# Snoworday/instance-segmentation-attention

Hardware: AMD Instinct MI355X
Metric: images/sec @256x256 bs=16 per GPU (higher is better)
Workload: dtype bf16; 1 GPU; train.py step fwd+bwd+update 256x256 bs=16/GPU (bf16); global_batch=16, parallelism=dp1, launch=hipGraph replay

## Files before the change

### instance-segmentation-attention_amd/csrc/common.hpp

```cpp
#pragma once
#include <hip/hip_runtime.h>
#include <stdint.h>
#include "../../include/isa_kernels.h"

typedef __bf16 bf16_t;
typedef __bf16 bf16x8 __attribute__((ext_vector_type(8)));
typedef __bf16 bf16x4 __attribute__((ext_vector_type(4)));
typedef float f32x4 __attribute__((ext_vector_type(4)));
typedef float f32x16 __attribute__((ext_vector_type(16)));

#define ISA_WAVE 64
#define ISA_STAT_R 8

static inline hipStream_t as_stream(void* s) { return reinterpret_cast<hipStream_t>(s); }

static inline int launch_status() {
    return hipGetLastError() == hipSuccess ? ISA_OK : ISA_ELAUNCH;
}

static inline bool tensor_ok(const isa_tensor* t, int align_elems) {
    if (!t || !t->data || t->n <= 0 || t->h <= 0 || t->w <= 0 || t->c <= 0 || t->ld < t->c) return false;
    if (t->dtype != ISA_F32 && t->dtype != ISA_BF16) return false;
    if (align_elems > 1) {
        size_t esz = t->dtype == ISA_F32 ? 4 : 2;
        if ((reinterpret_cast<uintptr_t>(t->data) % (align_elems * esz)) != 0) return false;
        if (t->ld % align_elems) return false;
    }
    return true;
}

template <typename T> struct st;
template <> struct st<float> {
    static constexpr int dtype = ISA_F32;
    static __device__ __forceinline__ float ld(const float* p) { return *p; }
    static __device__ __forceinline__ void stv(float* p, float v) { *p = v; }
};
template <> struct st<bf16_t> {
    static constexpr int dtype = ISA_BF16;
    static __device__ __forceinline__ float ld(const bf16_t* p) { return (float)*p; }
    static __device__ __forceinline__ void stv(bf16_t* p, float v) { *p = (bf16_t)v; }
};

template <typename T> __device__ __forceinline__ void load8(const T* p, float (&v)[8]);
template <> __device__ __forceinline__ void load8<float>(const float* p, float (&v)[8]) {
    f32x4 a = *reinterpret_cast<const f32x4*>(p), b = *reinterpret_cast<const f32x4*>(p + 4);
#pragma unroll
    for (int i = 0; i < 4; ++i) { v[i] = a[i]; v[4 + i] = b[i]; }
}
template <> __device__ __forceinline__ void load8<bf16_t>(const bf16_t* p, float (&v)[8]) {
    bf16x8 a = *reinterpret_cast<const bf16x8*>(p);
#pragma unroll
    for (int i = 0; i < 8; ++i) v[i] = (float)a[i];
}
template <typename T> __device__ __forceinline__ void store8(T* p, const float (&v)[8]);
template <> __device__ __forceinline__ void store8<float>(float* p, const float (&v)[8]) {
    f32x4 a, b;
#pragma unroll
    for (int i = 0; i < 4; ++i) { a[i] = v[i]; b[i] = v[4 + i]; }
    *reinterpret_cast<f32x4*>(p) = a;
    *reinterpret_cast<f32x4*>(p + 4) = b;
}
template <> __device__ __forceinline__ void store8<bf16_t>(bf16_t* p, const float (&v)[8]) {
    bf16x8 a;
#pragma unroll
    for (int i = 0; i < 8; ++i) a[i] = (bf16_t)v[i];
    *reinterpret_cast<bf16x8*>(p) = a;
}

template <typename T> __device__ __forceinline__ void load8g(const T* p, float (&v)[8], int nv) {
    if (nv >= 8) { load8<T>(p, v); return; }
#pragma unroll
    for (int i = 0; i < 8; ++i) v[i] = i < nv ? st<T>::ld(p + i) : 0.f;
}
template <typename T> __device__ __forceinline__ void store8g(T* p, const float (&v)[8], int nv) {
    if (nv >= 8) { store8<T>(p, v); return; }
#pragma unroll
    for (int i = 0; i < 8; ++i) if (i < nv) st<T>::stv(p + i, v[i]);
}

template <int CLS> __device__ __forceinline__ float row_fold(float v) {
    static_assert(CLS == 4 || CLS == 8, "lane classes per row");
    if constexpr (CLS == 4) v += __int_as_float(__builtin_amdgcn_update_dpp(0, __float_as_int(v), 0x124, 0xF, 0xF, false));
    v += __int_as_float(__builtin_amdgcn_update_dpp(0, __float_as_int(v), 0x128, 0xF, 0xF, false));
    return v;
}

__device__ __forceinline__ float act_apply(float z, int act) {
    switch (act) {
        case ISA_ACT_RELU:  return fmaxf(z, 0.f);
        case ISA_ACT_RELU6: return fminf(fmaxf(z, 0.f), 6.f);
        case ISA_ACT_LEAKY: return z > 0.f ? z : 0.01f * z;
        case ISA_ACT_TANH:  return tanhf(z);
        default:            return z;
    }
}
__device__ __forceinline__ float act_grad(float z, int act) {
    switch (act) {
        case ISA_ACT_RELU:  return z > 0.f ? 1.f : 0.f;
        case ISA_ACT_RELU6: return (z > 0.f && z < 6.f) ? 1.f : 0.f;
        case ISA_ACT_LEAKY: return z > 0.f ? 1.f : 0.01f;
        case ISA_ACT_TANH:  { float t = tanhf(z); return 1.f - t * t; }
        default:            return 1.f;
    }
}

constexpr int ACT_RT = -1;
template <int ACT> __device__ __forceinline__ float act_t(float z, int rt) {
    if constexpr (ACT == ISA_ACT_RELU6) return __builtin_amdgcn_fmed3f(z, 0.f, 6.f);
    else if constexpr (ACT == ISA_ACT_NONE) return z;
    else if constexpr (ACT == ISA_ACT_LEAKY) return z > 0.f ? z : 0.01f * z;
    else return act_apply(z, rt);
}
template <int ACT> __device__ __forceinline__ float act_grad_t(float z, int rt) {
    if constexpr (ACT == ISA_ACT_RELU6) return (z > 0.f && z < 6.f) ? 1.f : 0.f;
    else if constexpr (ACT == ISA_ACT_NONE) return 1.f;
    else if constexpr (ACT == ISA_ACT_LEAKY) return z > 0.f ? 1.f : 0.01f;
    else return act_grad(z, rt);
}

struct ProDev {
    const float* scale; const float* shift; const float* bscale; int act;
};
static inline ProDev make_pro(const isa_pro* p) {
    ProDev d{nullptr, nullptr, nullptr, ISA_ACT_NONE};
    if (p) { d.scale = p->scale; d.shift = p->shift; d.bscale = p->bscale; d.act = p->act; }
    return d;
}
static inline bool pro_trivial(const ProDev& p) {
    return !p.scale && !p.shift && !p.bscale && p.act == ISA_ACT_NONE;
}

struct FinDev {
    const float *stats, *gamma, *beta; float *rm, *rv, *scale, *shift, *mean, *invstd;
    float count, momentum, eps; int repeat;
};
static inline FinDev make_fin(const isa_pro* p) {
    FinDev f{}; f.repeat = 1;
    if (p && p->fin) {
        const isa_bn_fin* q = p->fin;
        f = FinDev{q->stats, q->gamma, q->beta, q->running_mean, q->running_var, q->scale, q->shift, q->mean, q->invstd,
                   q->count, q->momentum, q->eps, q->repeat < 1 ? 1 : q->repeat};
    }
    return f;
}
static inline bool fin_valid(const isa_pro* p) {
    return !p || !p->fin || (p->fin->stats && p->fin->scale && p->fin->shift && p->fin->scale == p->scale && p->fin->shift == p->shift);
}
int fin_standalone(const isa_pro* p, int c, int groups, hipStream_t s);

__device__ __forceinline__ void bn_fin_channel(const FinDev& f, int i, int c, int groups, bool all_groups, int gsel,
                                               float* tab, int tab_ld) {
    const float g = f.gamma ? f.gamma[i] : 1.f, b = f.beta ? f.beta[i] : 0.f;
    const bool run = all_groups || !f.stats;
    float rmi = (run && f.rm) ? f.rm[i] : 0.f, rvi = (run && f.rv) ? f.rv[i] : 0.f;
    const int g0 = all_groups ? 0 : gsel, g1 = all_groups ? groups : gsel + 1;
    for (int gi = g0; gi < g1; ++gi) {
        float mean, var;
        if (f.stats) {
            const float* st = f.stats + (long)gi * ISA_STAT_R * 2 * c;
            float s1 = 0.f, s2 = 0.f;
// ... 115 lines not shown
```

### instance-segmentation-attention_amd/csrc/dwconv.hip

```cpp
#include "common.hpp"
#include <type_traits>

namespace {

__device__ __forceinline__ void lds_barrier() {
    __builtin_amdgcn_fence(__ATOMIC_RELEASE, "workgroup", "local");
    __builtin_amdgcn_s_barrier();
    __builtin_amdgcn_fence(__ATOMIC_ACQUIRE, "workgroup", "local");
}

constexpr int TH = 8, TW = 32, CB = 32, PS = 36;
constexpr int HALO = (TH + 2) * (TW + 2);

struct Dw2Params {
    const void* x; const void* w; const float* bias; void* y; const void* dy;
    int n, h, w_, c, ldx, ldy, ldd, wld;
    ProDev pro;
    float* stats; int accumulate;
    int tiles_x, tiles_y; long ntiles;
    float* ws; int csrc;
    int G;
    FinDev fin;
};

template <typename T> struct raw8;
template <> struct raw8<bf16_t> {
    bf16x8 v;
    __device__ __forceinline__ void load(const bf16_t* p) { v = *reinterpret_cast<const bf16x8*>(p); }
    __device__ __forceinline__ float get(int j) const { return (float)v[j]; }
    __device__ __forceinline__ void store(bf16_t* p) const { *reinterpret_cast<bf16x8*>(p) = v; }
    __device__ __forceinline__ void zero() { v = bf16x8{}; }
};
template <> struct raw8<float> {
    f32x4 a, b;
    __device__ __forceinline__ void load(const float* p) { a = *reinterpret_cast<const f32x4*>(p); b = *reinterpret_cast<const f32x4*>(p + 4); }
    __device__ __forceinline__ float get(int j) const { return j < 4 ? a[j] : b[j - 4]; }
    __device__ __forceinline__ void store(float* p) const { *reinterpret_cast<f32x4*>(p) = a; *reinterpret_cast<f32x4*>(p + 4) = b; }
    __device__ __forceinline__ void zero() { a = f32x4{}; b = f32x4{}; }
};

struct ProRegs { float sc[8], sh[8], bs[8]; };

template <bool HAS_PRO>
__device__ __forceinline__ void load_pro(const Dw2Params& p, ProRegs& r, int c0, int b) {
#pragma unroll
    for (int j = 0; j < 8; ++j) {
        const int c = min(c0 + j, p.c - 1);
        r.sc[j] = (HAS_PRO && p.pro.scale) ? p.pro.scale[c] : 1.f;
        r.sh[j] = (HAS_PRO && p.pro.shift) ? p.pro.shift[c] : 0.f;
        r.bs[j] = (HAS_PRO && p.pro.bscale) ? p.pro.bscale[(long)b * p.c + c] : 1.f;
    }
}

template <typename T, bool HAS_PRO, int ACT>
__device__ __forceinline__ void stage_tile(const Dw2Params& p, const ProRegs& r, float* tile, int b, int ty, int tx, int c_base) {
    const T* xin = reinterpret_cast<const T*>(p.x);
    const int cg = threadIdx.x & 3;
    const int c0 = c_base + cg * 8;
    const bool cok = c0 < p.c;
    constexpr int NIT = (HALO * 4 + 255) / 256;
    float v[NIT][8];
    bool ok[NIT];
#pragma unroll
    for (int it = 0; it < NIT; ++it) {
        const int pix = (threadIdx.x + it * 256) >> 2;
        const int rr = pix / (TW + 2), cc = pix - rr * (TW + 2);
        const int gy = ty * TH + rr - 1, gx = tx * TW + cc - 1;
        ok[it] = pix < HALO && cok && gy >= 0 && gy < p.h && gx >= 0 && gx < p.w_;
        if (ok[it]) load8<T>(xin + (((long)b * p.h + gy) * p.w_ + gx) * p.ldx + c0, v[it]);
    }
#pragma unroll
    for (int it = 0; it < NIT; ++it) {
        const int pix = (threadIdx.x + it * 256) >> 2;
        if (pix >= HALO) continue;
        f32x4 a, bb;
#pragma unroll
        for (int j = 0; j < 8; ++j) {
            float z = 0.f;
            if (ok[it]) {
                z = v[it][j];
                if constexpr (HAS_PRO) {
                    z = act_t<ACT>(fmaf(z, r.sc[j], r.sh[j]), p.pro.act);
                    if (p.pro.bscale) z *= r.bs[j];
                }
            }
            if (j < 4) a[j] = z; else bb[j - 4] = z;
        }
        *reinterpret_cast<f32x4*>(tile + pix * PS + cg * 8) = a;
        *reinterpret_cast<f32x4*>(tile + pix * PS + cg * 8 + 4) = bb;
    }
}

typedef float f32x2 __attribute__((ext_vector_type(2)));
__device__ __forceinline__ void fma8(const float (&x)[8], const float (&w)[8], float (&acc)[8]) {
#ifdef ISA_DW_SCALAR_FMA
#pragma unroll
    for (int j = 0; j < 8; ++j) acc[j] = __builtin_fmaf(x[j], w[j], acc[j]);
#else
#pragma unroll
    for (int j = 0; j < 8; j += 2) {
        const f32x2 r = __builtin_elementwise_fma(f32x2{x[j], x[j + 1]}, f32x2{w[j], w[j + 1]}, f32x2{acc[j], acc[j + 1]});
        acc[j] = r[0]; acc[j + 1] = r[1];
    }
#endif
}

__device__ __forceinline__ void ld8(const float* p, float (&v)[8]) {
    const f32x4 a = *reinterpret_cast<const f32x4*>(p), b = *reinterpret_cast<const f32x4*>(p + 4);
#pragma unroll
    for (int j = 0; j < 4; ++j) { v[j] = a[j]; v[4 + j] = b[j]; }
}

struct TileRange { long t0, end, step; };
__device__ __forceinline__ TileRange tile_range(long ntiles, int bx, int nbx) {
    if ((nbx & 7) == 0 && ntiles >= 64) {
        const int xcd = bx & 7, j = bx >> 3;
        const long chunk = (ntiles + 7) / 8;
        const long end = min(ntiles, (xcd + 1) * chunk);
        return TileRange{xcd * chunk + j, end, (long)(nbx >> 3)};
    }
    return TileRange{(long)bx, ntiles, (long)nbx};
}
// ... 885 lines not shown
```

### instance-segmentation-attention_amd/csrc/elementwise.hip

```cpp
#include "common.hpp"

namespace {

template <typename T>
__global__ void pack_kernel(const isa_pack_entry* tab, const int32_t* kmap, const float* src, T* dst) {
    const isa_pack_entry e = tab[blockIdx.y];
    const float* s = src + e.src_off;
    T* d = dst + e.dst_off;
    const int32_t* km = e.kmap_off >= 0 ? kmap + e.kmap_off : nullptr;
    long total;
    const int rows = e.rows;
    switch (e.kind) {
        case 0: case 1: total = (long)rows * e.taps * e.kp; break;
        case 2: total = (long)rows * e.kp; break;
        case 3: total = (long)rows * 4 * e.kp; break;
        default: total = (long)9 * rows; break;
    }
    for (long i = (long)blockIdx.x * blockDim.x + threadIdx.x; i < total; i += (long)gridDim.x * blockDim.x) {
        float v = 0.f;
        if (e.kind == 0) {
            const int kd = (int)(i % e.kp); long q = i / e.kp;
            const int t = (int)(q % e.taps); const int n = (int)(q / e.taps);
            const int k = km ? km[kd] : (kd < e.k ? kd : -1);
            if (k >= 0) v = s[((long)n * e.k + k) * e.taps + t];
        } else if (e.kind == 1) {
            const int nd = (int)(i % e.kp); long q = i / e.kp;
            const int t = (int)(q % e.taps); const int kd = (int)(q / e.taps);
            const int k = km ? km[kd] : kd;
            if (k >= 0 && nd < e.n) v = s[((long)nd * e.k + k) * e.taps + (e.taps - 1 - t)];
        } else if (e.kind == 2) {
            const int kd = (int)(i % e.kp); const int row = (int)(i / e.kp);
            const int co_n = e.n;
            const int qd = row / co_n, co = row - qd * co_n;
            const int k = km ? km[kd] : (kd < e.k ? kd : -1);
            if (k >= 0) v = s[((long)k * co_n + co) * 4 + qd];
        } else if (e.kind == 3) {
            const int cod = (int)(i % e.kp); long q = i / e.kp;
            const int qd = (int)(q % 4); const int kd = (int)(q / 4);
            const int k = km ? km[kd] : kd;
            if (k >= 0 && cod < e.n) v = s[((long)k * e.n + cod) * 4 + qd];
        } else {
            const int cd = (int)(i % rows); const int t = (int)(i / rows);
            const int c = km ? km[cd] : (cd < e.n ? cd : -1);
            if (c >= 0) v = s[(long)c * 9 + (e.kind == 5 ? 8 - t : t)];
        }
        d[i] = (T)v;
    }
}

__global__ void bn_finalize_kernel(FinDev f, int c, int groups) {
    for (int i = blockIdx.x * blockDim.x + threadIdx.x; i < c; i += gridDim.x * blockDim.x)
        bn_fin_channel(f, i, c, groups, true, 0, nullptr, 0);
}

constexpr int BN_UPD_CHUNK = 64;
struct BnUpdChunk { isa_bn_upd d[BN_UPD_CHUNK]; };
__global__ __launch_bounds__(256) void bn_running_update_kernel(BnUpdChunk ch, float momentum) {
    const isa_bn_upd u = ch.d[blockIdx.x];
    const int c = u.c;
    for (int i = threadIdx.x; i < c; i += 256) {
        float s1 = 0.f, s2 = 0.f;
#pragma unroll
        for (int r = 0; r < ISA_STAT_R; ++r) { s1 += u.stats[r * 2 * c + i]; s2 += u.stats[r * 2 * c + c + i]; }
        const float mean = s1 / u.count;
        const float var = fmaxf(s2 / u.count - mean * mean, 0.f);
        u.running_mean[i] = (1.f - momentum) * u.running_mean[i] + momentum * mean;
        u.running_var[i] = (1.f - momentum) * u.running_var[i] + momentum * var * (u.count / fmaxf(u.count - 1.f, 1.f));
    }
}

struct View { void* data; int n, h, w, c, ld; };
static inline View mkview(const isa_tensor* t) { return View{t->data, t->n, t->h, t->w, t->c, t->ld}; }

struct BnBwdParams {
    View dt, y, dy;
    const float *scale, *shift, *mean, *invstd, *bscale, *gamma, *red;
    float* out_red; float* dgamma; float* dbeta;
    float inv_count; int act, train;
    long pixels; int cg;
    int groups;
};

struct Walk { int cg, sh; long pixels; };
static inline Walk mkwalk(int c, long pixels) {
    Walk w; w.cg = (c + 7) / 8; w.sh = 0;
    while ((1 << w.sh) < w.cg) ++w.sh;
    if (w.sh > 8) w.sh = 8;
    w.pixels = pixels; return w;
}
static inline int walk_grid(const Walk& w, int iters = 1) { return grid_cap(cdiv(w.pixels, (long)(256 >> w.sh) * iters)); }

template <typename T, bool APPLY, int ACT>
__global__ __launch_bounds__(256) void bn_bwd_kernel(BnBwdParams p, Walk wk) {
    extern __shared__ float red[];
    const int C = p.y.c;
    if (p.groups > 1 && blockIdx.z) {
        const long g = blockIdx.z, gp = g * wk.pixels;
        p.dt.data = reinterpret_cast<T*>(p.dt.data) + gp * p.dt.ld;
        p.y.data = reinterpret_cast<T*>(p.y.data) + gp * p.y.ld;
        if (APPLY) p.dy.data = reinterpret_cast<T*>(p.dy.data) + gp * p.dy.ld;
        p.scale = goff(p.scale, g * C); p.shift = goff(p.shift, g * C); p.mean = goff(p.mean, g * C);
        p.invstd = goff(p.invstd, g * C);
        p.bscale = goff(p.bscale, g * (wk.pixels / ((long)p.y.h * p.y.w)) * C);
        p.red = goff(p.red, g * ISA_STAT_R * 2 * C); p.out_red = goff(p.out_red, g * ISA_STAT_R * 2 * C);
    }
    if (!APPLY) {
        for (int i = threadIdx.x; i < 2 * C; i += 256) red[i] = 0.f;
        __syncthreads();
    } else if (p.red) {
        const int cw = 8 << wk.sh;
        for (int cb = blockIdx.y * cw; cb < C; cb += gridDim.y * cw) {
            for (int i = threadIdx.x; i < 2 * cw; i += 256) {
                const int which = i / cw, c = cb + (i - which * cw);
                if (c >= C) continue;
                float s = 0.f;
#pragma unroll
                for (int r = 0; r < ISA_STAT_R; ++r) s += p.red[r * 2 * C + which * C + c];
                red[which * C + c] = s;
                if (blockIdx.x == 0) {
                    if (which == 1 && p.dgamma) atomicAdd(p.dgamma + c, s);
                    if (which == 0 && p.dbeta) atomicAdd(p.dbeta + c, s);
                }
            }
        }
        __syncthreads();
    }
    const int ppb = 256 >> wk.sh;
    const int psub = threadIdx.x >> wk.sh;
    const unsigned hw = (unsigned)p.y.h * (unsigned)p.y.w;
    for (int cgi = (blockIdx.y << wk.sh) + (threadIdx.x & ((1 << wk.sh) - 1)); cgi < wk.cg; cgi += (gridDim.y << wk.sh)) {
        const int c0 = cgi * 8;
        const int nv = min(8, C - c0);
        float sc[8], sh[8], mu[8], is[8], k0[8], k1[8], s0[8], s1[8];
#pragma unroll
        for (int j = 0; j < 8; ++j) {
            const int c = min(c0 + j, C - 1);
            sc[j] = p.scale ? p.scale[c] : 1.f;
            sh[j] = p.shift ? p.shift[c] : 0.f;
            mu[j] = p.mean ? p.mean[c] : 0.f;
            is[j] = p.invstd ? p.invstd[c] : 1.f;
            k0[j] = (APPLY && p.train) ? red[c] * p.inv_count : 0.f;
            k1[j] = (APPLY && p.train) ? red[C + c] * p.inv_count : 0.f;
            s0[j] = 0.f; s1[j] = 0.f;
        }
        const long step = (long)gridDim.x * ppb;
        for (long pix = (long)blockIdx.x * ppb + psub; pix < wk.pixels; pix += step) {
            float dt[8], yv[8], out[8];
            load8g<T>(reinterpret_cast<const T*>(p.dt.data) + pix * p.dt.ld + c0, dt, nv);
            load8g<T>(reinterpret_cast<const T*>(p.y.data) + pix * p.y.ld + c0, yv, nv);
            const float* bs = p.bscale ? p.bscale + (long)((unsigned)pix / hw) * C : nullptr;
#pragma unroll
            for (int j = 0; j < 8; ++j) {
                const float z = fmaf(yv[j], sc[j], sh[j]);
                float dz = dt[j] * act_grad_t<ACT>(z, p.act);
                if (bs) dz *= bs[min(c0 + j, C - 1)];
                const float yh = (yv[j] - mu[j]) * is[j];
                if (!APPLY) { s0[j] += dz; s1[j] += dz * yh; }
                else out[j] = sc[j] * (dz - k0[j] - yh * k1[j]);
            }
            if (APPLY) store8g<T>(reinterpret_cast<T*>(p.dy.data) + pix * p.dy.ld + c0, out, nv);
        }
        if (!APPLY) {
            const int lane = threadIdx.x & 63;
            if (wk.sh < 6) {
#pragma unroll
                for (int j = 0; j < 8; ++j) {
                    for (int off = 1 << wk.sh; off < 64; off <<= 1) {
                        s0[j] += __shfl_xor(s0[j], off, 64); s1[j] += __shfl_xor(s1[j], off, 64);
                    }
                }
            }
            if (wk.sh >= 6 || (lane >> wk.sh) == 0) {
#pragma unroll
                for (int j = 0; j < 8; ++j)
                    if (j < nv) { atomicAdd(&red[c0 + j], s0[j]); atomicAdd(&red[C + c0 + j], s1[j]); }
            }
        }
    }
    if (!APPLY) {
        __syncthreads();
        float* rep = p.out_red + (blockIdx.x & (ISA_STAT_R - 1)) * 2 * C;
        for (int i = threadIdx.x; i < 2 * C; i += 256)
            if (red[i] != 0.f) atomicAdd(rep + i, red[i]);
    }
}

struct MatParams { View x, res, res2, out; ProDev pro; const float* oscale; long pixels; int cg; int has_res, has_res2; int groups, bcast; FinDev fin; };
template <typename T, int ACT>
__global__ __launch_bounds__(256) void materialize_kernel(MatParams p, Walk wk) {
    const int C = p.x.c;
    __shared__ float fin_tab[2 * ISA_FIN_MAX_C];
    const bool fin = bn_fin_inline<256>(p.fin, C, p.bcast ? 1 : p.groups, p.bcast ? 0 : (int)blockIdx.z, fin_tab, ISA_FIN_MAX_C,
                                        threadIdx.x);
    if (p.groups > 1 && blockIdx.z) {
        const long g = blockIdx.z, gp = g * wk.pixels;
        const long gimg = g * (wk.pixels / ((long)p.x.h * p.x.w)) * C;
        p.out.data = reinterpret_cast<T*>(p.out.data) + gp * p.out.ld;
        if (p.has_res2) p.res2.data = reinterpret_cast<T*>(p.res2.data) + gp * p.res2.ld;
        p.oscale = goff(p.oscale, gimg);
        if (!p.bcast) {
            p.x.data = reinterpret_cast<T*>(p.x.data) + gp * p.x.ld;
            if (p.has_res) p.res.data = reinterpret_cast<T*>(p.res.data) + gp * p.res.ld;
            p.pro.scale = goff(p.pro.scale, g * C); p.pro.shift = goff(p.pro.shift, g * C);
            p.pro.bscale = goff(p.pro.bscale, gimg);
        }
    }
    const int ppb = 256 >> wk.sh;
    const int psub = threadIdx.x >> wk.sh;
    const unsigned hw = (unsigned)p.x.h * (unsigned)p.x.w;
    for (int cgi = threadIdx.x & ((1 << wk.sh) - 1); cgi < wk.cg; cgi += (1 << wk.sh)) {
        const int c0 = cgi * 8;
        const int nv = min(8, C - c0);
        float sc[8], sh[8];
#pragma unroll
        for (int j = 0; j < 8; ++j) {
            const int c = min(c0 + j, C - 1);
            sc[j] = fin ? fin_tab[c] : (p.pro.scale ? p.pro.scale[c] : 1.f);
            sh[j] = fin ? fin_tab[ISA_FIN_MAX_C + c] : (p.pro.shift ? p.pro.shift[c] : 0.f);
        }
        const bool per_image = p.pro.bscale || p.oscale;
        const long step = (long)gridDim.x * ppb;
        for (long pix = (long)blockIdx.x * ppb + psub; pix < wk.pixels; pix += step) {
            float v[8];
            load8g<T>(reinterpret_cast<const T*>(p.x.data) + pix * p.x.ld + c0, v, nv);
            const long bofs = per_image ? (long)((unsigned)pix / hw) * C : 0;
#pragma unroll
            for (int j = 0; j < 8; ++j) v[j] = act_t<ACT>(fmaf(v[j], sc[j], sh[j]), p.pro.act);
            if (p.pro.bscale) {
#pragma unroll
                for (int j = 0; j < 8; ++j) v[j] *= p.pro.bscale[bofs + min(c0 + j, C - 1)];
            }
            if (p.has_res) {
                float rr[8];
                load8g<T>(reinterpret_cast<const T*>(p.res.data) + pix * p.res.ld + c0, rr, nv);
#pragma unroll
                for (int j = 0; j < 8; ++j) v[j] += rr[j];
            }
            if (p.has_res2) {
                float rr[8];
                load8g<T>(reinterpret_cast<const T*>(p.res2.data) + pix * p.res2.ld + c0, rr, nv);
#pragma unroll
                for (int j = 0; j < 8; ++j) v[j] += rr[j];
            }
            if (p.oscale) {
#pragma unroll
                for (int j = 0; j < 8; ++j) v[j] *= p.oscale[bofs + min(c0 + j, C - 1)];
            }
            store8g<T>(reinterpret_cast<T*>(p.out.data) + pix * p.out.ld + c0, v, nv);
        }
    }
}

struct AxpyParams { View src, dst; float alpha; int accumulate; long pixels; };
template <typename T>
__global__ __launch_bounds__(256) void axpy_kernel(AxpyParams p) {
    const int C = p.src.c;
    const long items = p.pixels * C;
    for (long i = (long)blockIdx.x * 256 + threadIdx.x; i < items; i += (long)gridDim.x * 256) {
        const int c = (int)(i % C); const long pix = i / C;
        float v = p.alpha == 0.f ? 0.f : p.alpha * st<T>::ld(reinterpret_cast<const T*>(p.src.data) + pix * p.src.ld + c);
        T* d = reinterpret_cast<T*>(p.dst.data) + pix * p.dst.ld + c;
        if (p.accumulate) v += st<T>::ld(d);
        st<T>::stv(d, v);
    }
}
template <typename T>
__global__ __launch_bounds__(256) void axpy8_kernel(AxpyParams p) {
    const int cg = p.src.c / 8;
    const long items = p.pixels * cg;
    for (long i = (long)blockIdx.x * 256 + threadIdx.x; i < items; i += (long)gridDim.x * 256) {
        const int c0 = (int)(i % cg) * 8; const long pix = i / cg;
        float v[8] = {0, 0, 0, 0, 0, 0, 0, 0};
        if (p.alpha != 0.f) load8<T>(reinterpret_cast<const T*>(p.src.data) + pix * p.src.ld + c0, v);
        T* d = reinterpret_cast<T*>(p.dst.data) + pix * p.dst.ld + c0;
        if (p.accumulate) {
            float o[8]; load8<T>(d, o);
#pragma unroll
            for (int j = 0; j < 8; ++j) v[j] = fmaf(p.alpha, v[j], o[j]);
        } else {
#pragma unroll
            for (int j = 0; j < 8; ++j) v[j] *= p.alpha;
        }
        store8<T>(d, v);
    }
}

struct PoolParams { View x, y; int accumulate; };
template <typename T, bool BWD>
__global__ __launch_bounds__(256) void avgpool2_kernel(PoolParams p) {
    const View big = BWD ? p.y : p.x, small = BWD ? p.x : p.y;
    const int cg = small.c / 8;
    const long items = (long)small.n * small.h * small.w * cg;
    for (long i = (long)blockIdx.x * 256 + threadIdx.x; i < items; i += (long)gridDim.x * 256) {
        const int c0 = (int)(i % cg) * 8; long q = i / cg;
        const int xs = (int)(q % small.w); q /= small.w;
        const int ys = (int)(q % small.h); const int b = (int)(q / small.h);
        T* sp = reinterpret_cast<T*>(small.data) + (((long)b * small.h + ys) * small.w + xs) * small.ld + c0;
        T* bp = reinterpret_cast<T*>(big.data) + (((long)b * big.h + 2 * ys) * big.w + 2 * xs) * big.ld + c0;
        if (!BWD) {
            float a[8], acc[8] = {0, 0, 0, 0, 0, 0, 0, 0};
#pragma unroll
            for (int d = 0; d < 4; ++d) {
                load8<T>(bp + ((long)(d >> 1) * big.w + (d & 1)) * big.ld, a);
#pragma unroll
                for (int j = 0; j < 8; ++j) acc[j] += a[j];
            }
#pragma unroll
            for (int j = 0; j < 8; ++j) acc[j] *= 0.25f;
            store8<T>(sp, acc);
        } else {
            float g[8];
            load8<T>(sp, g);
#pragma unroll
            for (int j = 0; j < 8; ++j) g[j] *= 0.25f;
#pragma unroll
            for (int d = 0; d < 4; ++d) {
                T* dp = bp + ((long)(d >> 1) * big.w + (d & 1)) * big.ld;
                float o[8];
                if (p.accumulate) {
                    load8<T>(dp, o);
#pragma unroll
                    for (int j = 0; j < 8; ++j) o[j] += g[j];
                } else {
#pragma unroll
                    for (int j = 0; j < 8; ++j) o[j] = g[j];
                }
                store8<T>(dp, o);
            }
        }
    }
}
// ... 184 lines not shown
}

static inline bool same_shape(const isa_tensor* a, const isa_tensor* b) {
    return a->n == b->n && a->h == b->h && a->w == b->w && a->c == b->c && a->dtype == b->dtype;
}

}

#define DISPATCH_T(dtype, CALL_BF16, CALL_F32) \
    do { if ((dtype) == ISA_BF16) { CALL_BF16; } else { CALL_F32; } } while (0)

extern "C" int isa_pack_weights(const isa_pack_entry* table_dev, int32_t n_entries,
                                const int32_t* kmap_dev, const float* src_base, void* dst_base,
                                int32_t dst_dtype, void* stream) {
    if (!table_dev || n_entries <= 0 || !src_base || !dst_base) return ISA_EINVAL;
    dim3 grid(32, n_entries);
    DISPATCH_T(dst_dtype,
        hipLaunchKernelGGL(pack_kernel<bf16_t>, grid, dim3(256), 0, as_stream(stream), table_dev, kmap_dev, src_base, (bf16_t*)dst_base),
        hipLaunchKernelGGL(pack_kernel<float>, grid, dim3(256), 0, as_stream(stream), table_dev, kmap_dev, src_base, (float*)dst_base));
    return launch_status();
}

extern "C" int isa_bn_finalize(const float* stats, float count, const float* gamma,
                               const float* beta, float* running_mean, float* running_var,
                               float momentum, float eps, float* scale, float* shift,
                               float* mean, float* invstd, int32_t c, int32_t groups, int32_t repeat, void* stream) {
    if (c <= 0 || !scale || !shift || (!stats && (!running_mean || !running_var))) return ISA_EINVAL;
    if (groups < 1) groups = 1;
    if (repeat < 1) repeat = 1;
    if (!stats && groups != 1) return ISA_EINVAL;
    const FinDev f{stats, gamma, beta, running_mean, running_var, scale, shift, mean, invstd, count, momentum, eps, repeat};
    hipLaunchKernelGGL(bn_finalize_kernel, dim3(cdiv(c, 256)), dim3(256), 0, as_stream(stream), f, c, groups);
    return launch_status();
}

int fin_standalone(const isa_pro* p, int c, int groups, hipStream_t s) {
    if (!p || !p->fin) return ISA_OK;
    if (!fin_valid(p) || c <= 0) return ISA_EINVAL;
    hipLaunchKernelGGL(bn_finalize_kernel, dim3(cdiv(c, 256)), dim3(256), 0, s, make_fin(p), c, groups < 1 ? 1 : groups);
    return launch_status();
}

extern "C" int isa_bn_running_update(const isa_bn_upd* upd, int32_t n, float momentum, void* stream) {
    if (n < 0 || (n > 0 && !upd)) return ISA_EINVAL;
    for (int i = 0; i < n; ++i)
        if (!upd[i].stats || !upd[i].running_mean || !upd[i].running_var || upd[i].c <= 0 || !(upd[i].count > 0)) return ISA_EINVAL;
    for (int i0 = 0; i0 < n; i0 += BN_UPD_CHUNK) {
        BnUpdChunk ch{};
        const int m = n - i0 < BN_UPD_CHUNK ? n - i0 : BN_UPD_CHUNK;
        for (int i = 0; i < m; ++i) ch.d[i] = upd[i0 + i];
        hipLaunchKernelGGL(bn_running_update_kernel, dim3(m), dim3(256), 0, as_stream(stream), ch, momentum);
        if (launch_status() != ISA_OK) return ISA_ELAUNCH;
    }
    return ISA_OK;
}

static int bn_bwd_common(const isa_tensor* dt, const isa_tensor* y, const isa_tensor* dy,
                         BnBwdParams& p, bool apply, void* stream) {
    if (!tensor_ok(dt, 8) || !tensor_ok(y, 8) || !same_shape(dt, y)) return ISA_EINVAL;
    p.dt = mkview(dt); p.y = mkview(y);
    if (apply) { if (!tensor_ok(dy, 8) || !same_shape(dy, y)) return ISA_EINVAL; p.dy = mkview(dy); }
    const int G = tensor_groups(y);
    if (y->n % G) return ISA_EINVAL;
    p.groups = G;
    p.pixels = (long)(y->n / G) * y->h * y->w; p.cg = (y->c + 7) / 8;
    if (p.pixels * G >= (1L << 32)) return ISA_EINVAL;
    Walk wk = mkwalk(y->c, p.pixels);
    int gy = 1, grid;
    if (wk.cg > 16) {
        wk.sh = 2; gy = (wk.cg + 3) / 4;
        const long trips = cdiv(p.pixels, 64);
        grid = (int)(apply ? (trips + 1) / 2 : (trips + 3) / 4);
        const int cap = apply ? 512 : 128;
        if (grid > cap) grid = cap;
        if (grid < 1) grid = 1;
    } else {
        const long per = 256 >> wk.sh;
        int iters = 16;
        if (cdiv(p.pixels, per * 16) < 512) { iters = (int)(p.pixels / (per * 512)); if (iters < 2) iters = 2; }
        grid = walk_grid(wk, iters);
        if (!apply && grid > 1024) grid = 1024;
    }
    const size_t lds = 2 * (size_t)y->c * 4;
#define BN_BWD_LAUNCH(AP, ACTV) \
    DISPATCH_T(y->dtype, \
        hipLaunchKernelGGL((bn_bwd_kernel<bf16_t, AP, ACTV>), dim3(grid, gy, G), dim3(256), lds, as_stream(stream), p, wk), \
        hipLaunchKernelGGL((bn_bwd_kernel<float, AP, ACTV>), dim3(grid, gy, G), dim3(256), lds, as_stream(stream), p, wk))
    if (apply) {
        if (p.act == ISA_ACT_RELU6) BN_BWD_LAUNCH(true, ISA_ACT_RELU6);
        else if (p.act == ISA_ACT_NONE) BN_BWD_LAUNCH(true, ISA_ACT_NONE);
        else BN_BWD_LAUNCH(true, ACT_RT);
    } else {
        if (p.act == ISA_ACT_RELU6) BN_BWD_LAUNCH(false, ISA_ACT_RELU6);
        else if (p.act == ISA_ACT_NONE) BN_BWD_LAUNCH(false, ISA_ACT_NONE);
        else BN_BWD_LAUNCH(false, ACT_RT);
    }
#undef BN_BWD_LAUNCH
    return launch_status();
}

extern "C" int isa_bn_bwd_reduce(const isa_tensor* dt, const isa_tensor* y, const float* scale,
                                 const float* shift, const float* mean, const float* invstd,
                                 int32_t act, const float* bscale, float* red, void* stream) {
    if (!red) return ISA_EINVAL;
    BnBwdParams p{};
    p.scale = scale; p.shift = shift; p.mean = mean; p.invstd = invstd; p.bscale = bscale;
    p.act = act; p.out_red = red; p.train = 1;
    return bn_bwd_common(dt, y, nullptr, p, false, stream);
}

extern "C" int isa_bn_bwd_apply(const isa_tensor* dt, const isa_tensor* y, const float* scale,
                                const float* shift, const float* mean, const float* invstd,
                                int32_t act, const float* bscale, const float* gamma,
                                const float* red, float count, int32_t train,
                                const isa_tensor* dy, float* dgamma, float* dbeta, void* stream) {
    if (train && !red) return ISA_EINVAL;
    BnBwdParams p{};
    p.scale = scale; p.shift = shift; p.mean = mean; p.invstd = invstd; p.bscale = bscale;
    p.gamma = gamma; p.red = red; p.inv_count = count > 0 ? 1.f / count : 0.f;
    p.act = act; p.train = train; p.dgamma = dgamma; p.dbeta = dbeta;
    return bn_bwd_common(dt, y, dy, p, true, stream);
}

extern "C" int isa_affine_act_res(const isa_tensor* x, const isa_pro* pro, const isa_tensor* res,
                                  const isa_tensor* res2, const float* oscale,
                                  const isa_tensor* out, void* stream) {
    if (!tensor_ok(x, 8) || !tensor_ok(out, 8)) return ISA_EINVAL;
    const int G = tensor_groups(out);
    const bool bcast = G > 1 && out->n == G * x->n && tensor_groups(x) == 1;
    if (bcast) {
        if (x->h != out->h || x->w != out->w || x->c != out->c || x->dtype != out->dtype) return ISA_EINVAL;
    } else if (!same_shape(x, out)) return ISA_EINVAL;
    if (out->n % G) return ISA_EINVAL;
    if (res && (!tensor_ok(res, 8) || !same_shape(res, x))) return ISA_EINVAL;
    if (res2 && (!tensor_ok(res2, 8) || !same_shape(res2, out))) return ISA_EINVAL;
    MatParams p{};
    p.x = mkview(x); p.out = mkview(out); p.pro = make_pro(pro); p.has_res = res != nullptr;
    p.has_res2 = res2 != nullptr; p.oscale = oscale;
    if (res) p.res = mkview(res);
    if (res2) p.res2 = mkview(res2);
    p.groups = G; p.bcast = bcast;
    p.pixels = (long)(out->n / G) * x->h * x->w; p.cg = (x->c + 7) / 8;
    if (p.pixels * G >= (1L << 32)) return ISA_EINVAL;
    if (pro && pro->fin) {
        if (!fin_valid(pro) || (!bcast && tensor_groups(x) != G)) return ISA_EINVAL;
        if (x->c <= ISA_FIN_MAX_C) p.fin = make_fin(pro);
        else if (int rc = fin_standalone(pro, x->c, tensor_groups(x), as_stream(stream))) return rc;
    }
    const Walk wk = mkwalk(x->c, p.pixels);
    const dim3 grid(walk_grid(wk), 1, G);
    if (p.pro.act == ISA_ACT_NONE)
        DISPATCH_T(x->dtype,
            hipLaunchKernelGGL((materialize_kernel<bf16_t, ISA_ACT_NONE>), grid, dim3(256), 0, as_stream(stream), p, wk),
            hipLaunchKernelGGL((materialize_kernel<float, ISA_ACT_NONE>), grid, dim3(256), 0, as_stream(stream), p, wk));
    else
        DISPATCH_T(x->dtype,
            hipLaunchKernelGGL((materialize_kernel<bf16_t, ACT_RT>), grid, dim3(256), 0, as_stream(stream), p, wk),
            hipLaunchKernelGGL((materialize_kernel<float, ACT_RT>), grid, dim3(256), 0, as_stream(stream), p, wk));
    return launch_status();
}

extern "C" int isa_axpy(const isa_tensor* src, const isa_tensor* dst, float alpha,
                        int32_t accumulate, void* stream) {
    if (!tensor_ok(src, 1) || !tensor_ok(dst, 1) || !same_shape(src, dst)) return ISA_EINVAL;
    AxpyParams p{mkview(src), mkview(dst), alpha, accumulate, (long)src->n * src->h * src->w};
    const bool vec = tensor_ok(src, 8) && tensor_ok(dst, 8) && src->c % 8 == 0;
    const int grid = grid_cap(cdiv(p.pixels * (vec ? src->c / 8 : src->c), 256));
    if (vec)
        DISPATCH_T(src->dtype,
            hipLaunchKernelGGL(axpy8_kernel<bf16_t>, dim3(grid), dim3(256), 0, as_stream(stream), p),
            hipLaunchKernelGGL(axpy8_kernel<float>, dim3(grid), dim3(256), 0, as_stream(stream), p));
    else
        DISPATCH_T(src->dtype,
            hipLaunchKernelGGL(axpy_kernel<bf16_t>, dim3(grid), dim3(256), 0, as_stream(stream), p),
            hipLaunchKernelGGL(axpy_kernel<float>, dim3(grid), dim3(256), 0, as_stream(stream), p));
    return launch_status();
}

extern "C" int isa_avgpool2(const isa_tensor* x, const isa_tensor* y, void* stream) {
    if (!tensor_ok(x, 8) || !tensor_ok(y, 8) || x->dtype != y->dtype || x->c != y->c || x->c % 8 ||
        x->n != y->n || x->h != 2 * y->h || x->w != 2 * y->w) return ISA_EINVAL;
    PoolParams p{mkview(x), mkview(y), 0};
    const int grid = grid_cap(cdiv((long)y->n * y->h * y->w * (y->c / 8), 256));
    DISPATCH_T(x->dtype,
        hipLaunchKernelGGL((avgpool2_kernel<bf16_t, false>), dim3(grid), dim3(256), 0, as_stream(stream), p),
        hipLaunchKernelGGL((avgpool2_kernel<float, false>), dim3(grid), dim3(256), 0, as_stream(stream), p));
    return launch_status();
}

extern "C" int isa_avgpool2_bwd(const isa_tensor* dy, const isa_tensor* dx, int32_t accumulate,
                                void* stream) {
    if (!tensor_ok(dy, 8) || !tensor_ok(dx, 8) || dy->dtype != dx->dtype || dy->c != dx->c ||
        dy->c % 8 || dy->n != dx->n || dx->h != 2 * dy->h || dx->w != 2 * dy->w) return ISA_EINVAL;
    PoolParams p{mkview(dy), mkview(dx), accumulate};
    const int grid = grid_cap(cdiv((long)dy->n * dy->h * dy->w * (dy->c / 8), 256));
    DISPATCH_T(dy->dtype,
        hipLaunchKernelGGL((avgpool2_kernel<bf16_t, true>), dim3(grid), dim3(256), 0, as_stream(stream), p),
        hipLaunchKernelGGL((avgpool2_kernel<float, true>), dim3(grid), dim3(256), 0, as_stream(stream), p));
    return launch_status();
}

extern "C" int isa_avgpool3(const isa_tensor* x, const isa_tensor* mask, const isa_tensor* y,
                            int32_t accumulate, void* stream) {
    if (!tensor_ok(x, 1) || !tensor_ok(y, 1) || !same_shape(x, y)) return ISA_EINVAL;
    if (mask && (!tensor_ok(mask, 1) || mask->n != x->n || mask->h != x->h || mask->w != x->w ||
                 mask->dtype != x->dtype)) return ISA_EINVAL;
    Pool3Params p{mkview(x), mask ? mkview(mask) : View{}, mkview(y), mask != nullptr, accumulate};
    const long vec_items = (long)y->n * y->h * y->w * (y->c / 8);
    const bool aligned = (reinterpret_cast<uintptr_t>(x->data) % 16 == 0) && (reinterpret_cast<uintptr_t>(y->data) % 16 == 0);
    if (y->c % 8 == 0 && x->ld % 8 == 0 && y->ld % 8 == 0 && aligned && vec_items < (1L << 31)) {
        const int gridv = grid_cap(cdiv(vec_items, 256), 256 * 16);
        DISPATCH_T(x->dtype,
            hipLaunchKernelGGL(avgpool3_vec_kernel<bf16_t>, dim3(gridv), dim3(256), 0, as_stream(stream), p),
            hipLaunchKernelGGL(avgpool3_vec_kernel<float>, dim3(gridv), dim3(256), 0, as_stream(stream), p));
        return launch_status();
    }
    const int grid = grid_cap(cdiv((long)y->n * y->h * y->w * y->c, 256));
    DISPATCH_T(x->dtype,
        hipLaunchKernelGGL(avgpool3_kernel<bf16_t>, dim3(grid), dim3(256), 0, as_stream(stream), p),
        hipLaunchKernelGGL(avgpool3_kernel<float>, dim3(grid), dim3(256), 0, as_stream(stream), p));
    return launch_status();
}

extern "C" int isa_chan_mean(const isa_tensor* x, const isa_pro* pro, float* out, void* stream) {
    if (!tensor_ok(x, 8) || x->c % 8 || !out || x->n % tensor_groups(x)) return ISA_EINVAL;
    if (pro && pro->fin) { if (int rc = fin_standalone(pro, x->c, tensor_groups(x), as_stream(stream))) return rc; }
    MeanParams p{mkview(x), make_pro(pro), out, 1.f / ((float)x->h * x->w), tensor_groups(x)};
    const long items = (long)x->h * x->w * (x->c / 8);
    dim3 grid(grid_cap(cdiv(items, 256), 128), x->n);
    DISPATCH_T(x->dtype,
        hipLaunchKernelGGL(chan_mean_kernel<bf16_t>, grid, dim3(256), x->c * 4, as_stream(stream), p),
        hipLaunchKernelGGL(chan_mean_kernel<float>, grid, dim3(256), x->c * 4, as_stream(stream), p));
    return launch_status();
}

extern "C" int isa_se_fc(const float* mean, const float* w1, const float* b1, const float* w2,
                         const float* b2, int32_t n, int32_t c, int32_t hidden, float* hid,
                         float* gate, void* stream) {
    if (!mean || !w1 || !b1 || !w2 || !b2 || !gate || n <= 0 || c <= 0 || hidden <= 0) return ISA_EINVAL;
    hipLaunchKernelGGL(se_fc_kernel, dim3(n), dim3(64), (c + hidden) * 4, as_stream(stream), mean, w1, b1,
                       w2, b2, c, hidden, hid, gate);
// ... 43 lines not shown
```

Baseline: 662.7 images/s.

## Unroll streaming BN-backward and materialize loops with batched loads and per-image scale caching

Restructures the BN backward and materialize elementwise kernels so each thread issues the loads for several strided pixels before computing on any of them, with a scheduling barrier to keep the loads grouped. This is meant to raise memory-level parallelism in these bandwidth-bound kernels. Per-image scale rows (bscale and oscale) are now held in registers and reloaded only when the image index changes, and a template flag selects this path at launch. Waves-per-EU attributes are added to steer occupancy. The added register pressure and code size could lower occupancy or increase spills.

```diff
diff --git a/instance-segmentation-attention_amd/csrc/common.hpp b/instance-segmentation-attention_amd/csrc/common.hpp
--- a/instance-segmentation-attention_amd/csrc/common.hpp
+++ b/instance-segmentation-attention_amd/csrc/common.hpp
@@ -76,6 +76,43 @@
     if (nv >= 8) { store8<T>(p, v); return; }
 #pragma unroll
     for (int i = 0; i < 8; ++i) if (i < nv) st<T>::stv(p + i, v[i]);
+}
+
+template <typename T> struct raw8;
+template <> struct raw8<bf16_t> {
+    bf16x8 v;
+    __device__ __forceinline__ void load(const bf16_t* p) { v = *reinterpret_cast<const bf16x8*>(p); }
+    __device__ __forceinline__ float get(int j) const { return (float)v[j]; }
+    __device__ __forceinline__ void store(bf16_t* p) const { *reinterpret_cast<bf16x8*>(p) = v; }
+    __device__ __forceinline__ void zero() { v = bf16x8{}; }
+    __device__ __forceinline__ void pack(const float (&f)[8]) {
+#pragma unroll
+        for (int i = 0; i < 8; ++i) v[i] = (bf16_t)f[i];
+    }
+    __device__ __forceinline__ void store1(bf16_t* p, int j) const { p[j] = v[j]; }
+};
+template <> struct raw8<float> {
+    f32x4 a, b;
+    __device__ __forceinline__ void load(const float* p) { a = *reinterpret_cast<const f32x4*>(p); b = *reinterpret_cast<const f32x4*>(p + 4); }
+    __device__ __forceinline__ float get(int j) const { return j < 4 ? a[j] : b[j - 4]; }
+    __device__ __forceinline__ void store(float* p) const { *reinterpret_cast<f32x4*>(p) = a; *reinterpret_cast<f32x4*>(p + 4) = b; }
+    __device__ __forceinline__ void zero() { a = f32x4{}; b = f32x4{}; }
+    __device__ __forceinline__ void pack(const float (&f)[8]) {
+#pragma unroll
+        for (int i = 0; i < 4; ++i) { a[i] = f[i]; b[i] = f[4 + i]; }
+    }
+    __device__ __forceinline__ void store1(float* p, int j) const { p[j] = get(j); }
+};
+
+template <typename T> __device__ __forceinline__ raw8<T> load8raw(const T* p) { raw8<T> r; r.load(p); return r; }
+template <typename T> __device__ __forceinline__ void unpack8m(const raw8<T>& r, float (&v)[8], int nv) {
+#pragma unroll
+    for (int i = 0; i < 8; ++i) v[i] = i < nv ? r.get(i) : 0.f;
+}
+template <typename T> __device__ __forceinline__ void store8raw(T* p, const raw8<T>& r, int nv) {
+    if (nv >= 8) { r.store(p); return; }
+#pragma unroll
+    for (int i = 0; i < 8; ++i) if (i < nv) r.store1(p, i);
 }
 
 template <int CLS> __device__ __forceinline__ float row_fold(float v) {
diff --git a/instance-segmentation-attention_amd/csrc/dwconv.hip b/instance-segmentation-attention_amd/csrc/dwconv.hip
--- a/instance-segmentation-attention_amd/csrc/dwconv.hip
+++ b/instance-segmentation-attention_amd/csrc/dwconv.hip
@@ -23,21 +23,6 @@
     FinDev fin;
 };
 
-template <typename T> struct raw8;
-template <> struct raw8<bf16_t> {
-    bf16x8 v;
-    __device__ __forceinline__ void load(const bf16_t* p) { v = *reinterpret_cast<const bf16x8*>(p); }
-    __device__ __forceinline__ float get(int j) const { return (float)v[j]; }
-    __device__ __forceinline__ void store(bf16_t* p) const { *reinterpret_cast<bf16x8*>(p) = v; }
-    __device__ __forceinline__ void zero() { v = bf16x8{}; }
-};
-template <> struct raw8<float> {
-    f32x4 a, b;
-    __device__ __forceinline__ void load(const float* p) { a = *reinterpret_cast<const f32x4*>(p); b = *reinterpret_cast<const f32x4*>(p + 4); }
-    __device__ __forceinline__ float get(int j) const { return j < 4 ? a[j] : b[j - 4]; }
-    __device__ __forceinline__ void store(float* p) const { *reinterpret_cast<f32x4*>(p) = a; *reinterpret_cast<f32x4*>(p + 4) = b; }
-    __device__ __forceinline__ void zero() { a = f32x4{}; b = f32x4{}; }
-};
 
 struct ProRegs { float sc[8], sh[8], bs[8]; };
 
diff --git a/instance-segmentation-attention_amd/csrc/elementwise.hip b/instance-segmentation-attention_amd/csrc/elementwise.hip
--- a/instance-segmentation-attention_amd/csrc/elementwise.hip
+++ b/instance-segmentation-attention_amd/csrc/elementwise.hip
@@ -90,8 +90,24 @@
 }
 static inline int walk_grid(const Walk& w, int iters = 1) { return grid_cap(cdiv(w.pixels, (long)(256 >> w.sh) * iters)); }
 
-template <typename T, bool APPLY, int ACT>
-__global__ __launch_bounds__(256) void bn_bwd_kernel(BnBwdParams p, Walk wk) {
+constexpr int STREAM_U_REDUCE = 2, STREAM_U_APPLY = 2, STREAM_U_MAT = 2;
+template <typename T> constexpr int stream_u(int u) { return sizeof(T) == 2 ? u : (u > 1 ? u / 2 : 1); }
+#define STREAM_WAVES(n) __attribute__((amdgpu_waves_per_eu(n, n)))
+
+typedef float f32x4u __attribute__((ext_vector_type(4), aligned(4)));
+__device__ __forceinline__ void load_row8(const float* row, float (&v)[8], int nv) {
+    if (nv >= 8) {
+        const f32x4u a = *reinterpret_cast<const f32x4u*>(row), b = *reinterpret_cast<const f32x4u*>(row + 4);
+#pragma unroll
+        for (int j = 0; j < 4; ++j) { v[j] = a[j]; v[4 + j] = b[j]; }
+        return;
+    }
+#pragma unroll
+    for (int j = 0; j < 8; ++j) v[j] = j < nv ? row[j] : 0.f;
+}
+
+template <typename T, bool APPLY, int ACT, bool PI>
+__global__ __launch_bounds__(256) STREAM_WAVES((!APPLY && ACT == ISA_ACT_NONE) ? 5 : 4) void bn_bwd_kernel(BnBwdParams p, Walk wk) {
     extern __shared__ float red[];
     const int C = p.y.c;
     if (p.groups > 1 && blockIdx.z) {
@@ -144,21 +160,57 @@
             s0[j] = 0.f; s1[j] = 0.f;
         }
         const long step = (long)gridDim.x * ppb;
-        for (long pix = (long)blockIdx.x * ppb + psub; pix < wk.pixels; pix += step) {
-            float dt[8], yv[8], out[8];
-            load8g<T>(reinterpret_cast<const T*>(p.dt.data) + pix * p.dt.ld + c0, dt, nv);
-            load8g<T>(reinterpret_cast<const T*>(p.y.data) + pix * p.y.ld + c0, yv, nv);
-            const float* bs = p.bscale ? p.bscale + (long)((unsigned)pix / hw) * C : nullptr;
-#pragma unroll
-            for (int j = 0; j < 8; ++j) {
-                const float z = fmaf(yv[j], sc[j], sh[j]);
-                float dz = dt[j] * act_grad_t<ACT>(z, p.act);
-                if (bs) dz *= bs[min(c0 + j, C - 1)];
-                const float yh = (yv[j] - mu[j]) * is[j];
-                if (!APPLY) { s0[j] += dz; s1[j] += dz * yh; }
-                else out[j] = sc[j] * (dz - k0[j] - yh * k1[j]);
-            }
-            if (APPLY) store8g<T>(reinterpret_cast<T*>(p.dy.data) + pix * p.dy.ld + c0, out, nv);
+        const long pix_first = (long)blockIdx.x * ppb + psub;
+        float bsr[8];
+        unsigned bimg = 0;
+        if (PI && pix_first < wk.pixels) {
+            bimg = (unsigned)pix_first / hw;
+            load_row8(p.bscale + (long)bimg * C + c0, bsr, nv);
+        }
+        constexpr int U = PI ? 1 : stream_u<T>(APPLY ? STREAM_U_APPLY : STREAM_U_REDUCE);
+        for (long pix0 = pix_first; pix0 < wk.pixels; pix0 += U * step) {
+            raw8<T> rdt[U], ry[U], rout[U];
+            unsigned pixu[U]; bool ok[U];
+#pragma unroll
+            for (int u = 0; u < U; ++u) {
+                const long pix = pix0 + u * step;
+                ok[u] = pix < wk.pixels;
+                pixu[u] = (unsigned)(ok[u] ? pix : pix0);
+            }
+#pragma unroll
+            for (int u = 0; u < U; ++u) {
+                rdt[u] = load8raw<T>(reinterpret_cast<const T*>(p.dt.data) + (long)pixu[u] * p.dt.ld + c0);
+                ry[u] = load8raw<T>(reinterpret_cast<const T*>(p.y.data) + (long)pixu[u] * p.y.ld + c0);
+            }
+            __builtin_amdgcn_sched_barrier(0);
+#pragma unroll
+            for (int u = 0; u < U; ++u) {
+                float dt[8], yv[8], out[8];
+                unpack8m<T>(rdt[u], dt, nv);
+                unpack8m<T>(ry[u], yv, nv);
+                if (PI) {
+                    const unsigned img = pixu[u] / hw;
+                    if (img != bimg) {
+                        bimg = img;
+                        load_row8(p.bscale + (long)img * C + c0, bsr, nv);
+                    }
+                }
+#pragma unroll
+                for (int j = 0; j < 8; ++j) {
+                    const float z = fmaf(yv[j], sc[j], sh[j]);
+                    float dz = dt[j] * act_grad_t<ACT>(z, p.act);
+                    if (PI) dz *= bsr[j];
+                    const float yh = (yv[j] - mu[j]) * is[j];
+                    if (!APPLY) { if (!ok[u]) dz = 0.f; s0[j] += dz; s1[j] += dz * yh; }
+                    else out[j] = sc[j] * (dz - k0[j] - yh * k1[j]);
+                }
+                if (APPLY) rout[u].pack(out);
+            }
+            if (APPLY) {
+#pragma unroll
+                for (int u = 0; u < U; ++u)
+                    store8raw<T>(reinterpret_cast<T*>(p.dy.data) + (long)pixu[u] * p.dy.ld + c0, rout[u], nv);
+            }
         }
         if (!APPLY) {
             const int lane = threadIdx.x & 63;
@@ -186,8 +238,8 @@
 }
 
 struct MatParams { View x, res, res2, out; ProDev pro; const float* oscale; long pixels; int cg; int has_res, has_res2; int groups, bcast; FinDev fin; };
-template <typename T, int ACT>
-__global__ __launch_bounds__(256) void materialize_kernel(MatParams p, Walk wk) {
+template <typename T, int ACT, bool PI>
+__global__ __launch_bounds__(256) STREAM_WAVES(sizeof(T) == 2 ? 5 : 4) void materialize_kernel(MatParams p, Walk wk) {
     const int C = p.x.c;
     __shared__ float fin_tab[2 * ISA_FIN_MAX_C];
     const bool fin = bn_fin_inline<256>(p.fin, C, p.bcast ? 1 : p.groups, p.bcast ? 0 : (int)blockIdx.z, fin_tab, ISA_FIN_MAX_C,
@@ -218,35 +270,73 @@
             sc[j] = fin ? fin_tab[c] : (p.pro.scale ? p.pro.scale[c] : 1.f);
             sh[j] = fin ? fin_tab[ISA_FIN_MAX_C + c] : (p.pro.shift ? p.pro.shift[c] : 0.f);
         }
-        const bool per_image = p.pro.bscale || p.oscale;
         const long step = (long)gridDim.x * ppb;
-        for (long pix = (long)blockIdx.x * ppb + psub; pix < wk.pixels; pix += step) {
-            float v[8];
-            load8g<T>(reinterpret_cast<const T*>(p.x.data) + pix * p.x.ld + c0, v, nv);
-            const long bofs = per_image ? (long)((unsigned)pix / hw) * C : 0;
-#pragma unroll
-            for (int j = 0; j < 8; ++j) v[j] = act_t<ACT>(fmaf(v[j], sc[j], sh[j]), p.pro.act);
-            if (p.pro.bscale) {
-#pragma unroll
-                for (int j = 0; j < 8; ++j) v[j] *= p.pro.bscale[bofs + min(c0 + j, C - 1)];
-            }
+        const long pix_first = (long)blockIdx.x * ppb + psub;
+        float bsr[8], osr[8];
+        unsigned bimg = 0;
+        auto load_rows = [&](unsigned img) {
+            bimg = img;
+            const long bofs = (long)img * C + c0;
+            if (p.pro.bscale) load_row8(p.pro.bscale + bofs, bsr, nv);
+            if (p.oscale) load_row8(p.oscale + bofs, osr, nv);
+        };
+        if (PI && pix_first < wk.pixels) load_rows((unsigned)pix_first / hw);
+        constexpr int U = PI ? 1 : stream_u<T>(STREAM_U_MAT);
+        for (long pix0 = pix_first; pix0 < wk.pixels; pix0 += U * step) {
+            raw8<T> rx[U], rr[U], rr2[U], rout[U];
+            unsigned pixu[U]; bool ok[U];
+#pragma unroll
+            for (int u = 0; u < U; ++u) {
+                const long pix = pix0 + u * step;
+                ok[u] = pix < wk.pixels;
+                pixu[u] = (unsigned)(ok[u] ? pix : pix0);
+            }
+#pragma unroll
+            for (int u = 0; u < U; ++u) rx[u] = load8raw<T>(reinterpret_cast<const T*>(p.x.data) + (long)pixu[u] * p.x.ld + c0);
             if (p.has_res) {
-                float rr[8];
-                load8g<T>(reinterpret_cast<const T*>(p.res.data) + pix * p.res.ld + c0, rr, nv);
-#pragma unroll
-                for (int j = 0; j < 8; ++j) v[j] += rr[j];
+#pragma unroll
+                for (int u = 0; u < U; ++u) rr[u] = load8raw<T>(reinterpret_cast<const T*>(p.res.data) + (long)pixu[u] * p.res.ld + c0);
             }
             if (p.has_res2) {
-                float rr[8];
-                load8g<T>(reinterpret_cast<const T*>(p.res2.data) + pix * p.res2.ld + c0, rr, nv);
-#pragma unroll
-                for (int j = 0; j < 8; ++j) v[j] += rr[j];
-            }
-            if (p.oscale) {
-#pragma unroll
-                for (int j = 0; j < 8; ++j) v[j] *= p.oscale[bofs + min(c0 + j, C - 1)];
-            }
-            store8g<T>(reinterpret_cast<T*>(p.out.data) + pix * p.out.ld + c0, v, nv);
+#pragma unroll
+                for (int u = 0; u < U; ++u) rr2[u] = load8raw<T>(reinterpret_cast<const T*>(p.res2.data) + (long)pixu[u] * p.res2.ld + c0);
+            }
+            __builtin_amdgcn_sched_barrier(0);
+#pragma unroll
+            for (int u = 0; u < U; ++u) {
+                float v[8];
+                unpack8m<T>(rx[u], v, nv);
+                if (PI) {
+                    const unsigned img = pixu[u] / hw;
+                    if (img != bimg) load_rows(img);
+                }
+#pragma unroll
+                for (int j = 0; j < 8; ++j) v[j] = act_t<ACT>(fmaf(v[j], sc[j], sh[j]), p.pro.act);
+                if (PI && p.pro.bscale) {
+#pragma unroll
+                    for (int j = 0; j < 8; ++j) v[j] *= bsr[j];
+                }
+                if (p.has_res) {
+                    float r[8];
+                    unpack8m<T>(rr[u], r, nv);
+#pragma unroll
+                    for (int j = 0; j < 8; ++j) v[j] += r[j];
+                }
+                if (p.has_res2) {
+                    float r[8];
+                    unpack8m<T>(rr2[u], r, nv);
+#pragma unroll
+                    for (int j = 0; j < 8; ++j) v[j] += r[j];
+                }
+                if (PI && p.oscale) {
+#pragma unroll
+                    for (int j = 0; j < 8; ++j) v[j] *= osr[j];
+                }
+                rout[u].pack(v);
+            }
+#pragma unroll
+            for (int u = 0; u < U; ++u)
+                store8raw<T>(reinterpret_cast<T*>(p.out.data) + (long)pixu[u] * p.out.ld + c0, rout[u], nv);
         }
     }
 }
@@ -597,10 +687,12 @@
         if (!apply && grid > 1024) grid = 1024;
     }
     const size_t lds = 2 * (size_t)y->c * 4;
+#define BN_BWD_LAUNCH_T(TT, AP, ACTV) \
+    do { if (p.bscale) hipLaunchKernelGGL((bn_bwd_kernel<TT, AP, ACTV, true>), dim3(grid, gy, G), dim3(256), lds, as_stream(stream), p, wk); \
+         else hipLaunchKernelGGL((bn_bwd_kernel<TT, AP, ACTV, false>), dim3(grid, gy, G), dim3(256), lds, as_stream(stream), p, wk); } while (0)
 #define BN_BWD_LAUNCH(AP, ACTV) \
     DISPATCH_T(y->dtype, \
-        hipLaunchKernelGGL((bn_bwd_kernel<bf16_t, AP, ACTV>), dim3(grid, gy, G), dim3(256), lds, as_stream(stream), p, wk), \
-        hipLaunchKernelGGL((bn_bwd_kernel<float, AP, ACTV>), dim3(grid, gy, G), dim3(256), lds, as_stream(stream), p, wk))
+        BN_BWD_LAUNCH_T(bf16_t, AP, ACTV), BN_BWD_LAUNCH_T(float, AP, ACTV))
     if (apply) {
         if (p.act == ISA_ACT_RELU6) BN_BWD_LAUNCH(true, ISA_ACT_RELU6);
         else if (p.act == ISA_ACT_NONE) BN_BWD_LAUNCH(true, ISA_ACT_NONE);
@@ -611,6 +703,7 @@
         else BN_BWD_LAUNCH(false, ACT_RT);
     }
 #undef BN_BWD_LAUNCH
+#undef BN_BWD_LAUNCH_T
     return launch_status();
 }
 
@@ -664,14 +757,13 @@
     }
     const Walk wk = mkwalk(x->c, p.pixels);
     const dim3 grid(walk_grid(wk), 1, G);
-    if (p.pro.act == ISA_ACT_NONE)
-        DISPATCH_T(x->dtype,
-            hipLaunchKernelGGL((materialize_kernel<bf16_t, ISA_ACT_NONE>), grid, dim3(256), 0, as_stream(stream), p, wk),
-            hipLaunchKernelGGL((materialize_kernel<float, ISA_ACT_NONE>), grid, dim3(256), 0, as_stream(stream), p, wk));
-    else
-        DISPATCH_T(x->dtype,
-            hipLaunchKernelGGL((materialize_kernel<bf16_t, ACT_RT>), grid, dim3(256), 0, as_stream(stream), p, wk),
-            hipLaunchKernelGGL((materialize_kernel<float, ACT_RT>), grid, dim3(256), 0, as_stream(stream), p, wk));
+    const bool pi = p.pro.bscale || p.oscale;
+#define MAT_LAUNCH(TT, ACTV) \
+    do { if (pi) hipLaunchKernelGGL((materialize_kernel<TT, ACTV, true>), grid, dim3(256), 0, as_stream(stream), p, wk); \
+         else hipLaunchKernelGGL((materialize_kernel<TT, ACTV, false>), grid, dim3(256), 0, as_stream(stream), p, wk); } while (0)
+    if (p.pro.act == ISA_ACT_NONE) DISPATCH_T(x->dtype, MAT_LAUNCH(bf16_t, ISA_ACT_NONE), MAT_LAUNCH(float, ISA_ACT_NONE));
+    else DISPATCH_T(x->dtype, MAT_LAUNCH(bf16_t, ACT_RT), MAT_LAUNCH(float, ACT_RT));
+#undef MAT_LAUNCH
     return launch_status();
 }
 
```

After: 692.6 images/s (median of 6 runs). 4.5% higher.
